# c0stya/trre

Measured on AMD Instinct MI355X. Metric: input GB/s (scan mode), higher is better.
Workload: dtype u8; 1 GPU; '[a:A-z:Z]' DFT scan over 8.000 GiB of synthetic printable lines per GPU (BASELINE.json configs[1] at north_star's size: >= 8 GiB); pattern=[a:A-z:Z], engine=dft, corpus=printable, bytes_per_gpu=8589934592, output_bytes_per_gpu=8589934592, kernel=bytemap, parallelism=line-sharded x1, one rank per GPU, no data-path collective

## Files before the change

### trre_amd/csrc/front.hpp

```cpp
#pragma once
#include <array>
#include <cstdint>
#include <memory>
#include <stdexcept>
#include <string>
#include <vector>

namespace trre {

enum : int {
    kOk = 0,
    kErrSyntax = -1,
    kErrUndefined = -2,
    kErrEpsCycle = -3,
    kErrTooBig = -4,
    kErrUnsupported = -5,
    kErrDevice = -6,
    kErrArg = -7,
    kErrDiverges = -8,
    kErrCapacity = -9
};

struct Error : std::runtime_error {
    int code;
// ... 118 lines not shown
private:
    struct Impl;
    std::unique_ptr<Impl> impl_;
};

struct StreamLimits {
    size_t max_states = 16384;
    size_t max_pending = 64;
    size_t max_out = 4096;
};
struct StreamTables {
    bool ok = false;
    bool bounded = false;
    uint32_t n_states = 0, n_cls = 0, flags = 0, max_out = 0;
    std::array<uint8_t, 256> cls{};
    std::vector<uint64_t> ent;
    std::vector<uint8_t> pool;
    std::vector<uint32_t> pending_len;
    bool lpw_ok = false;
    uint32_t lpw_delay = 0;
    std::vector<uint32_t> lpw;
    bool lpw2_ok = false;
    std::vector<uint32_t> lpw2;
    bool g16_ok = false;
    std::vector<uint32_t> g16;
    std::vector<uint32_t> mg;
    uint32_t mg_max = 0;
    bool p32_ok = false, p32_slow = false;
    std::vector<uint32_t> p32;
    bool fb_ok = false;
    uint32_t fb_states = 0, fb_dense = 0;
    uint32_t fb_start[3][2] = {};
    std::vector<uint64_t> fb_comb;
    std::vector<uint64_t> fb_lit;
    std::vector<uint32_t> fb_esc_slot;
    std::vector<uint32_t> fb_esc;
    std::vector<uint8_t> fb_pool;
    bool fb_copy_ok = false;
    std::vector<uint16_t> fb_lit_meta;
    bool fb_mark4_ok = false;
    uint32_t fb_pad = 0;
    uint32_t fb_start4[3] = {};
    std::vector<uint32_t> fb_comb4;
    std::vector<uint32_t> fb_dense4;
    std::vector<uint16_t> fb_dense_base;
};
// ... 96 lines not shown
```

### trre_amd/csrc/launch.hpp

```cpp
#pragma once
#include <cstdint>

namespace trre {

struct ScanArgs;
struct FbCopyArgs;
struct GenArgs;
struct GuardArgs;
struct LazyArgs;
struct OneArgs;
struct MapGenArgs;
struct RecArgs;
struct StrArgs;
struct MatchArgs;

constexpr int kEngineNft = 0, kEngineDft = 1;

int chunk_bytes(int engine, int mask_bytes);
int block_threads(int engine, int mask_bytes);

void launch_tile_kernel(int which, int engine, int mask_bytes, const ScanArgs& a, int64_t n_chunks, void* stream);
int direct_ent_lds_bytes();
int direct_block_threads();
void launch_direct_kernel(int which, bool ent_in_lds, const ScanArgs& a, int64_t lane_bytes, int64_t n_blocks, void* stream, int g16_bytes = 0,
                          int sym = 0, bool g16_slow = true);
int launch_one(const ScanArgs& a, const OneArgs& oa, void* stream, int g16_bytes, int sym, bool g16_slow);
int launch_mapgen(const ScanArgs& a, const MapGenArgs& oa, void* stream);
void launch_rev_sweep(const ScanArgs& a, int tab_bytes, int64_t lane_bytes, void* stream, bool packed);
void launch_rev_wide(const ScanArgs& a, int64_t lane_bytes, void* stream);
void launch_wide_fwd(int which, const ScanArgs& a, int64_t lane_bytes, int64_t n_blocks, void* stream);
void launch_lpw_kernel(int ent_bytes, bool wide, bool direct_ent_in_lds, const ScanArgs& a, int64_t lane_bytes, void* stream, int pair_bytes = 0);
void launch_fb_kernel(int which, const ScanArgs& a, const void* hdr, int64_t lane_bytes, int64_t n_chunks, void* stream);
bool fb_fits(const void* hdr);
void launch_fb_mark(const ScanArgs& a, const FbCopyArgs& ca, const void* hdr, int64_t lane_bytes, int64_t n_chunks, void* stream);
bool fb_copy_fits(const void* hdr);
void launch_fb_splice(const ScanArgs& a, const FbCopyArgs& ca, const void* hdr, int64_t lane_bytes, int64_t n_chunks, void* stream);
bool fb_splice_fits(const void* hdr);
void launch_gen(int which, const ScanArgs& a, const GenArgs& ga, int64_t lane_bytes, int64_t n_chunks, void* stream);
void launch_guard_probe(const ScanArgs& a, int64_t window, int64_t n_windows, uint64_t* flags, void* stream);
void launch_guard(bool out, const ScanArgs& a, const GuardArgs& ga, int64_t n_runs, int64_t slots, void* stream);
void launch_bt(int which, const ScanArgs& a, const GenArgs& ga, int64_t lane_bytes, int64_t n_chunks, int64_t pool_blocks, uint32_t budget, void* stream);
void launch_lazy(int which, const ScanArgs& a, const LazyArgs& la, int64_t lane_bytes, int64_t n_chunks, void* stream);
void launch_spec_verify(const ScanArgs& a, int64_t n_lanes, void* stream);
void launch_rev_verify(const ScanArgs& a, int64_t lane_bytes, void* stream, bool packed);
void launch_rev_repair(const ScanArgs& a, int64_t lane_bytes, void* stream, bool packed);
void launch_line_probe(const ScanArgs& a, int64_t window, uint32_t* out, void* stream);
void launch_chunk_scan(const uint64_t* total, uint64_t* base, int64_t n_chunks, void* stream);
void launch_bytemap(const ScanArgs& a, void* stream);
void launch_nul_eol(const uint8_t* in, int64_t n, const uint64_t* pos, uint64_t* eol, uint32_t count, void* stream);
int64_t rec_tile_bytes();
void launch_rec_check(const int64_t* off, int64_t nrec, int64_t n, uint32_t* status, void* stream);
void launch_rec_part(int side, const RecArgs& a, int64_t tiles, void* stream);
void launch_rec_stage(const RecArgs& a, int64_t tiles, void* stream);
void launch_rec_rank(const RecArgs& a, void* stream);
// ... 18 lines not shown
```

### trre_amd/csrc/runtime.cpp

```cpp
#include <hip/hip_runtime_api.h>

#include <cstdio>
#include <cstdlib>
#include <chrono>
#include <cstring>
#include <algorithm>
#include <atomic>
#include <condition_variable>
#include <functional>
#include <map>
#include <memory>
#include <mutex>
#include <string>
#include <thread>
#include <vector>

#include <sys/mman.h>

#include "../../include/trre_mi355x.h"
#include "device_blob.hpp"
#include "front.hpp"
#include "launch.hpp"
#include "switches.hpp"
#include "scan_block.hpp"
// ... 53 lines not shown
    *out = static_cast<uint8_t*>(m);
    return hipSuccess;
}
void pinned_put(uint8_t* p) {
    if (!p) return;
    size_t len = 0;
    {
        std::lock_guard<std::mutex> lk(g_pin_mu);
        auto it = g_pin_len.find(p);
        if (it == g_pin_len.end()) return;
        len = it->second;
        g_pin_len.erase(it);
    }
    (void)hipHostUnregister(p);
    ::munmap(p, len);
}

struct LaunchPlan {
    trre::ScanArgs args{};
    int64_t lane_bytes = 0, rev_lane_bytes = 0, n_chunks = 0;
    int threads = 0, sym_mode = 0;
    int g16 = 0;
    bool g16_slow = false, direct_ent_lds = false;
    bool direct = false;
    bool window = false, mapgen_on = false, use_exact = false;
};

struct Pending {
    bool active = false;
    int family = 0;
    int asked = 0;
    const uint8_t* d_in = nullptr;
    uint8_t* d_out = nullptr;
    const uint8_t* user_in = nullptr;
    bool aliased = false;
    size_t n = 0, cap = 0;
    hipStream_t stream = nullptr;
    bool launched = false;
    bool timed = false;
    int count = 0;
    const uint64_t* total_at = nullptr;
    bool patched = false;
    bool one = false;
    bool mapgen = false;
    bool exact = false;
    LaunchPlan plan;
// ... 184 lines not shown
    pred.push_back(t.to_final);
    put(b, 0, &h, 1);
    put(b, h.off_cons_mask, t.cons_mask.data(), 256);
    put(b, h.off_pred, pred.data(), pred.size());
    put(b, h.off_follow_off, t.follow_off.data(), t.follow_off.size());
    put(b, h.off_follow, t.follow.data(), t.follow.size());
    put(b, h.off_pool, t.pool.data(), t.pool.size());
}

void serialize_stream(const trre::StreamTables& t, std::vector<uint8_t>& b) {
    using namespace trre;
    StreamBlobHeader h{};
    h.magic = kMagicStream;
    h.n_states = t.n_states;
    h.n_cls = t.n_cls;
    h.flags = t.flags;
    h.max_out = t.max_out;
    size_t off = sizeof h;
    h.off_cls = (uint32_t)off; off += 256;
    h.off_ent = (uint32_t)off; h.ent_bytes = (uint32_t)(t.ent.size() * 8); off += t.ent.size() * 8;
    h.off_pool = (uint32_t)off; h.pool_bytes = (uint32_t)t.pool.size(); off += t.pool.size();
    off = align_up(off, 16);
    h.off_lpw = (uint32_t)off; h.lpw_bytes = (uint32_t)(t.lpw.size() * 4); h.lpw_delay = t.lpw_delay; off += t.lpw.size() * 4;
    off = align_up(off, 16);
    h.off_g16 = (uint32_t)off; h.g16_bytes = (uint32_t)(t.g16.size() * 4); off += t.g16.size() * 4;
    off = align_up(off, 16);
    h.off_p32 = (uint32_t)off; h.p32_bytes = (uint32_t)(t.p32.size() * 4); h.p32_slow = t.p32_slow ? 1u : 0u; off += t.p32.size() * 4;
    off = align_up(off, 16);
    h.off_lpw2 = (uint32_t)off; h.lpw2_bytes = (uint32_t)(t.lpw2.size() * 4); off += t.lpw2.size() * 4;
    off = align_up(off, 16);
    if (t.fb_ok) {
        h.fb_slots = (uint32_t)t.fb_comb.size(); h.off_fb_comb = (uint32_t)off; off = align_up(off + t.fb_comb.size() * 8, 16);
        h.fb_lits = (uint32_t)t.fb_lit.size(); h.off_fb_lit = (uint32_t)off; off = align_up(off + t.fb_lit.size() * 8, 16);
        h.fb_escs = (uint32_t)t.fb_esc_slot.size(); h.off_fb_esc_slot = (uint32_t)off; off = align_up(off + t.fb_esc_slot.size() * 4, 16);
        h.off_fb_esc = (uint32_t)off; off = align_up(off + t.fb_esc.size() * 4, 16);
        h.off_fb_pool = (uint32_t)off; off = align_up(off + t.fb_pool.size(), 16);
        if (t.fb_copy_ok) { h.off_fb_lit_meta = (uint32_t)off; off = align_up(off + t.fb_lit_meta.size() * 2, 16); }
        if (t.fb_mark4_ok) {
            h.fb4_slots = (uint32_t)t.fb_comb4.size(); h.off_fb_comb4 = (uint32_t)off; off = align_up(off + t.fb_comb4.size() * 4, 16);
            h.fb4_dense = (uint32_t)t.fb_dense_base.size(); h.off_fb_dense4 = (uint32_t)off; off = align_up(off + t.fb_dense4.size() * 4, 16);
            h.off_fb_dense_base = (uint32_t)off; off = align_up(off + t.fb_dense_base.size() * 2, 16);
            h.fb_pad = t.fb_pad;
            std::memcpy(h.fb_start4, t.fb_start4, sizeof h.fb_start4);
        }
        std::memcpy(h.fb_start, t.fb_start, sizeof h.fb_start);
    }
// ... 500 lines not shown
    pd.mapgen = true;
    return TRRE_OK;
}

int long_line_switch(trre_prog* p, ScanCtx* cx, int* family, const uint8_t* d_in, size_t n, size_t cap, hipStream_t stream) {
    const int exact_env = trre::switches().exact;
    const bool small_tables = (*family == TRRE_KERNEL_STREAM_LP && p->stt.g16_ok) || (*family == TRRE_KERNEL_GUIDED_LP && p->gt.fwd.g16_ok && !p->gt.wide);
    if (!small_tables || cx->exact_off || exact_env == 0 || cap < n) return TRRE_OK;
    if (cx->probe_in != d_in || cx->probe_n != n) {
        HIP_TRY(cx->d_probe.reserve(1, 16));
        uint32_t misses = 0;
        HIP_TRY(hipMemsetAsync(cx->d_probe, 0, 4, stream));
        trre::launch_line_probe(base_args(d_in, n), 32768, cx->d_probe, stream);
        HIP_TRY(hipMemcpyAsync(&misses, cx->d_probe, 4, hipMemcpyDeviceToHost, stream));
        HIP_TRY(hipStreamSynchronize(stream));
        cx->probe_in = d_in; cx->probe_n = n;
        cx->long_lines = misses != 0;
    }
    if (exact_env == 2 || cx->long_lines)
        *family = *family == TRRE_KERNEL_STREAM_LP ? TRRE_KERNEL_STREAM_GEN : TRRE_KERNEL_GUIDED_GEN;
    return TRRE_OK;
}

const trre::StreamTables& walked_tables(const trre_prog* p, int family) { return is_guided(family) ? p->gt.fwd : p->stt; }

LaunchPlan make_plan(const trre_prog* p, const DeviceState* st, const ScanCtx* cx, int family, const uint8_t* d_in, size_t n, uint8_t* d_out, size_t cap) {
    using namespace trre;
    const Switches& sw = switches();
    LaunchPlan pl;
    ScanArgs& args = pl.args;
    args = base_args(d_in, n, d_out);
    args.blob = is_stream(family) ? st->d_sblob : (is_guided(family) ? st->d_gblob : st->d_blob);
    const StreamTables& stt = walked_tables(p, family);
    args.status = cx->d_status;
    args.cap = cap;
    args.gscratch = cx->d_scratch.cap >= (n + 32) * (size_t)p->mask_bytes ? cx->d_scratch.p : nullptr;
    const bool backtrack = family == TRRE_KERNEL_BACKTRACK;
    const bool lazy = family == TRRE_KERNEL_DFT_LAZY;
    const int chunk = backtrack ? (int)kBtLaneBytes * 256 : lazy ? (int)kLazyLaneBytes * 256
                      : is_stream(family) ? 2048 * direct_block_threads() : chunk_bytes(p->engine, p->mask_bytes);
    pl.threads = backtrack || lazy ? 256 : is_stream(family) ? direct_block_threads() : block_threads(p->engine, p->mask_bytes);
    pl.n_chunks = (args.vend + chunk - 1) / chunk;
    pl.window = is_stream(family) && family == TRRE_KERNEL_STREAM_LP && p->stt.lpw_ok &&
                (reinterpret_cast<uintptr_t>(args.out_v0) & 15u) == 0;
    int64_t lane_auto = 2048;
    if (pl.window)
        while (lane_auto < 16384 && (int64_t)n / (lane_auto * 2) >= 524288) lane_auto *= 2;
    if ((family == TRRE_KERNEL_STREAM_GEN && (p->stt.g16_ok || p->stt.fb_ok)) || (is_guided(family) && !p->gt.wide))
        while (lane_auto < 8192 && (int64_t)n / (lane_auto * 2) >= 262144) lane_auto *= 2;
    pl.lane_bytes = sw.lane_bytes > 0 ? (sw.lane_bytes + 127) / 128 * 128 : lane_auto;
    pl.direct = is_stream(family) || is_guided(family);
    pl.rev_lane_bytes = sw.lane_bytes > 0 ? pl.lane_bytes : 2048;
    pl.direct_ent_lds = stt.ok && stt.ent.size() * 8 <= (size_t)direct_ent_lds_bytes();
    pl.g16_slow = (stt.flags & kFlagG16Slow) != 0;
    pl.g16 = stt.g16_ok && !sw.no_g16 ? (int)(align_up(stt.g16.size() * 4, 16) + stt.p32.size() * 4) : 0;
    pl.mapgen_on = stt.mg_max != 0 && (sw.mapgen < 0 ? !(stt.mg_max > 1u && cx->mapgen_dense) : sw.mapgen != 0) && !cx->mapgen_off && cx->mapgen_voids < 2;
    pl.sym_mode = !is_guided(family) ? 0 : (guided_sym_bits(*p) == 4 ? 2 : 1);
    if (pl.direct) pl.n_chunks = (args.vend + pl.lane_bytes * direct_block_threads() - 1) / (pl.lane_bytes * direct_block_threads());
    pl.use_exact = pl.g16 > 0 && !cx->exact_off && sw.exact != 0 && pl.lane_bytes % 128 == 0 && pl.rev_lane_bytes % 128 == 0 && !is_guided_wide(*p, family);
    return pl;
}


int route_lazy(trre_prog* p, DeviceState* st, ScanCtx* cx, LaunchPlan& pl, hipStream_t stream) {
    return lazy_round(p, st, cx, pl.args, pl.n_chunks, true, stream);
}
int route_backtrack(DeviceState* st, ScanCtx* cx, LaunchPlan& pl, hipStream_t stream) {
    using namespace trre;
    const BtTier& tier = kBtTiers[cx->bt_tier];
    const int64_t pool_blocks = pl.n_chunks < tier.pool_blocks ? pl.n_chunks : tier.pool_blocks;
    const uint32_t kBtFrames = tier.frames, kBtPathCap = tier.path_cap;
    const size_t need = (size_t)pool_blocks * 256 * ((size_t)kBtFrames * 16 + kBtPathCap);
    HIP_TRY(cx->d_scratch.reserve(need, need));
    GenArgs ga{};
    ga.stack = reinterpret_cast<uint32_t*>(cx->d_scratch.p);
    ga.path = cx->d_scratch + (size_t)pool_blocks * 256 * kBtFrames * 16;
    ga.frames = kBtFrames;
    ga.path_cap = kBtPathCap;
    pl.args.blob = st->d_nblob;
    const uint32_t budget = (uint32_t)switches().bt_budget.or_else(kBtBudget);
    launch_bt(1, pl.args, ga, kBtLaneBytes, pl.n_chunks, pool_blocks, budget, stream);
    launch_chunk_scan(cx->d_chunk_total, cx->d_chunk_base, pl.n_chunks, stream);
    launch_bt(2, pl.args, ga, kBtLaneBytes, pl.n_chunks, pool_blocks, budget, stream);
    return TRRE_OK;
}
int route_window(trre_prog* p, ScanCtx* cx, LaunchPlan& pl, hipStream_t stream) {
    using namespace trre;
    const int64_t n_lanes = (pl.args.vend + pl.lane_bytes - 1) / pl.lane_bytes;
    HIP_TRY(cx->d_redo.reserve((size_t)n_lanes, (size_t)(n_lanes + 1) * 4));
    HIP_TRY(hipMemsetAsync(cx->d_redo, 0, 4, stream));
    pl.args.redo = cx->d_redo;
    launch_lpw_kernel((int)(p->stt.lpw.size() * 4), p->stt.lpw_delay > 3, pl.direct_ent_lds, pl.args, pl.lane_bytes, stream,
                      p->stt.lpw2_ok && !switches().no_lpw_pair ? (int)(p->stt.lpw2.size() * 4) : 0);
    return TRRE_OK;
}
int route_wide_guided(ScanCtx* cx, LaunchPlan& pl, hipStream_t stream) {
    using namespace trre;
    launch_rev_wide(pl.args, pl.lane_bytes, stream);
    launch_wide_fwd(1, pl.args, pl.lane_bytes, pl.n_chunks, stream);
    launch_chunk_scan(cx->d_chunk_total, cx->d_chunk_base, pl.n_chunks, stream);
    launch_wide_fwd(2, pl.args, pl.lane_bytes, pl.n_chunks, stream);
    return TRRE_OK;
}
int route_lp_direct(trre_prog* p, int family, LaunchPlan& pl, hipStream_t stream) {
    using namespace trre;
    if (is_guided(family)) launch_rev_sweep(pl.args, (int)p->gt.n_rev * 256, pl.rev_lane_bytes, stream, pl.sym_mode == 2);
    pl.args.lp_emit = 1;
    launch_direct_kernel(2, pl.direct_ent_lds, pl.args, pl.lane_bytes, pl.n_chunks, stream, pl.g16, pl.sym_mode, pl.g16_slow);
    return TRRE_OK;
}
int route_large_table_copy(trre_prog* p, ScanCtx* cx, LaunchPlan& pl, hipStream_t stream) {
    using namespace trre;
    const Switches& sw = switches();
    uint32_t esc_max = 0;
    for (size_t k = 0; k + 3 < p->stt.fb_esc.size(); k += 4) esc_max = std::max(esc_max, p->stt.fb_esc[k + 1]);
    if (sw.no_fb_copy || sw.fb_emit || cx->patch_off || p->copy_form_off.load() || pl.lane_bytes % 64 != 0 || !fb_copy_fits(p->sblob.data()) ||
// ... 113 lines not shown
            hipStream_t stream) {
    Pending& pd = cx->pend;
    const bool batch = pd.active && pd.launched;
    if (pd.active && (pd.asked != family || pd.user_in != d_in || pd.d_out != d_out || pd.n != n || pd.cap != cap || pd.stream != stream))
        return fail(TRRE_E_ARG, "error: a different scan is still in flight on this device: call trre_scan_finish first");
    const int batch_count = batch ? pd.count : 0;
    const uint8_t* const user_in = d_in;
    const bool aliased = n && d_in == d_out;
    if (aliased) {
        const size_t a0 = reinterpret_cast<uintptr_t>(d_in) & 15u;
        if (!batch) {
            HIP_TRY(cx->d_snap.reserve(n + 16, n + 16));
            HIP_TRY(hipMemcpyAsync(cx->d_snap + a0, d_in, n, hipMemcpyDeviceToDevice, stream));
        }
        d_in = cx->d_snap + a0;
    }
    pd = Pending();
    pd.active = true;
    pd.count = batch_count;
    pd.family = family; pd.asked = family;
    pd.d_in = d_in; pd.d_out = d_out; pd.n = n; pd.cap = cap; pd.stream = stream;
    pd.user_in = user_in; pd.aliased = aliased;
    if (n == 0) return TRRE_OK;
    int rc = long_line_switch(p, cx, &family, d_in, n, cap, stream);
    if (rc) return rc;
    pd.family = family;
    if (family == TRRE_KERNEL_DFT_LAZY) { rc = lazy_ensure(p); if (rc) return rc; }
    LaunchPlan pl = make_plan(p, st, cx, family, d_in, n, d_out, cap);
    if (!is_gen(family) && cap < n) return TRRE_OK;
    if (is_gen(family)) {
        rc = ensure_workspace(cx, pl.n_chunks, pl.direct ? trre::direct_block_threads() : pl.threads);
        if (rc) return rc;
        pl.args.lane_counts = cx->d_lane_counts;
        pl.args.chunk_total = cx->d_chunk_total;
        pl.args.chunk_base = cx->d_chunk_base;
    }
    if (is_guided(family)) {
        const size_t need = ((size_t)((pl.args.vend + 63) & ~(int64_t)63) + 256) * (p->gt.wide ? 2 : 1);
        HIP_TRY(cx->d_sym.reserve(need, need));
        pl.args.rblob = st->d_rblob;
        pl.args.sym_v0 = cx->d_sym;
    }
    if (!batch) {
        HIP_TRY(hipMemsetAsync(cx->d_status, 0, 24, stream));
        if (p->profiling) HIP_TRY(hipEventRecord(cx->ev0, stream));
    }
    pd.timed = p->profiling;
// ... 1749 lines not shown
```

### trre_amd/csrc/scan_block.hpp

```cpp
#pragma once
#include <cstddef>
#include <cstdint>
#include <type_traits>

#include "device_blob.hpp"
#include "scan_core.hpp"

namespace trre {

struct alignas(16) U128 { uint32_t x, y, z, w; };


template <int THREADS_, int CHUNK_, int HALO_>
struct Geometry {
    static constexpr int THREADS = THREADS_;
    static constexpr int CHUNK = CHUNK_;
    static constexpr int HALO = HALO_;
    static constexpr int PRE = 16;
    static constexpr int TILE = PRE + CHUNK + HALO;
    static constexpr int TILE_ALLOC = TILE + 16;
    static constexpr int SUB = CHUNK / THREADS;
    static_assert(CHUNK % THREADS == 0 && TILE % 16 == 0, "geometry");
};

// ... 1710 lines not shown
    const uint32_t k = atomicAdd(a.redo, 1u);
#else
    const uint32_t k = a.redo[0]++;
#endif
    a.redo[1 + k] = (uint32_t)lane;
}

constexpr int kWtBlocks = 4;
constexpr int kWtPiece = 16 * kWtBlocks;
constexpr int kWtTile = 64 * kWtPiece;
constexpr int kWtOutRow = 128;
constexpr int kWtOutTile = 64 * kWtOutRow;

struct WtOutRow {
    uint8_t* row;
    uint32_t swz16;
    TRRE_HD uint8_t* slot(int b) const { return row + ((uint32_t)(b << 4) ^ swz16); }
};

TRRE_HD void lpw_classes(const LpwView& T, uint32_t w, uint32_t (&kk)[4]) {
    kk[0] = T.cls[w & 0xffu]; kk[1] = T.cls[(w >> 8) & 0xffu]; kk[2] = T.cls[(w >> 16) & 0xffu]; kk[3] = T.cls[w >> 24];
}

template <bool kCheckEnd, bool kWide>
TRRE_HD void wt_block(const LpwView& T, const U128& cur, uint32_t next_w, uint32_t (&kk)[4], int32_t rv, int32_t rhi, uint32_t& row,
                      uint32_t& win, uint32_t& win_hi, uint32_t& seen, uint32_t (&Rm)[4], uint32_t& done, int32_t& rend) {
    const uint32_t wd[5] = {cur.x, cur.y, cur.z, cur.w, next_w};
    uint32_t R = 0;
#pragma unroll
    for (int d = 0; d < 4; ++d) {
        uint32_t w = wd[d];
        const uint32_t kc[4] = {kk[0], kk[1], kk[2], kk[3]};
        lpw_classes(T, wd[d + 1], kk);
#pragma unroll
        for (int j = 0; j < 4; ++j) {
            const uint8_t* ep = reinterpret_cast<const uint8_t*>(T.ent) + row + (kc[j] << (kWide ? 5 : 4));
            const U128 e = *reinterpret_cast<const U128*>(ep);
            const uint32_t seq = perm_b32(w, e.z, e.w);
            if (!kWide) {
                win |= seq << (e.y & 63u);
                R = alignbit_b32(win, R, 8);
                win >>= 8;
            } else {
                const uint64_t e2 = *reinterpret_cast<const uint64_t*>(ep + 16);
                const uint32_t seq2 = perm_b32(w, (uint32_t)e2, (uint32_t)(e2 >> 32));
                uint64_t w64 = (uint64_t)win_hi << 32 | win;
                w64 |= ((uint64_t)seq2 << 32 | seq) << (e.y & 63u);
                R = alignbit_b32((uint32_t)w64, R, 8);
                w64 >>= 8;
                win = (uint32_t)w64;
                win_hi = (uint32_t)(w64 >> 32);
            }
            row = e.x;
            seen |= e.y;
            if (kCheckEnd) {
                const int32_t p1 = rv + 4 * d + j + 1;
                const uint32_t hit = ((e.y >> 6) & 1u) & (uint32_t)(p1 >= rhi) & (done ^ 1u);
                rend = hit ? p1 : rend;
                done |= hit;
            }
            w >>= 8;
        }
        Rm[d] = R;
        TRRE_PIN(seen);
        if (kCheckEnd) { TRRE_PIN(done); TRRE_PIN(rend); }
        TRRE_SCHED_FENCE();
    }
}

template <bool kCheckEnd>
TRRE_HD void wt_block_pair(const LpwView& T, const U128& cur, uint32_t next_w, uint32_t (&kk)[4], int32_t rv, int32_t rhi, uint32_t& row,
                           uint32_t& win, uint32_t& win_hi, uint32_t& seen, uint32_t (&Rm)[4], uint32_t& done, int32_t& rend) {
    const uint32_t wd[5] = {cur.x, cur.y, cur.z, cur.w, next_w};
    uint32_t R = 0;
#pragma unroll
    for (int d = 0; d < 4; ++d) {
        const uint32_t w = wd[d];
        const uint32_t kc[4] = {kk[0], kk[1], kk[2], kk[3]};
        lpw_classes(T, wd[d + 1], kk);
#pragma unroll
        for (int j = 0; j < 2; ++j) {
#if defined(__HIP_DEVICE_COMPILE__)
            const uint32_t col = __umul24(kc[2 * j], T.n_cls) + kc[2 * j + 1];
#else
            const uint32_t col = kc[2 * j] * T.n_cls + kc[2 * j + 1];
#endif
            const uint8_t* ep = reinterpret_cast<const uint8_t*>(T.ent) + row + (col << 5);
            const U128 e = *reinterpret_cast<const U128*>(ep);
            const uint64_t e2 = *reinterpret_cast<const uint64_t*>(ep + 16);
            const uint32_t w2 = w >> (16 * j);
            win |= perm_b32(w2, e.z, e.w);
            win_hi |= perm_b32(w2, (uint32_t)e2, (uint32_t)(e2 >> 32));
            R = alignbit_b32(win, R, 16);
            win = alignbit_b32(win_hi, win, 16);
            win_hi >>= 16;
            row = e.x;
            seen |= e.y;
            if (kCheckEnd) {
                const int32_t p1 = rv + 4 * d + 2 * j + 1;
// ... 542 lines not shown
```

### trre_amd/csrc/scan_kernels.hip

```cpp
#include <hip/hip_runtime.h>

#include <atomic>
#include <cstdlib>

#include "launch.hpp"
#include "switches.hpp"
#include "scan_block.hpp"
#include "splice_block.hpp"
#include "one_block.hpp"
#include "gen_block.hpp"
#include "lazy_block.hpp"
#include "guard_block.hpp"
#include "records_block.hpp"
#include "pass_block.hpp"

namespace trre {
namespace {

template <class G, class Engine>
struct Carve {
    static constexpr int kTab = (Engine::kLdsBytes + 15) & ~15;
    static constexpr int kMask = G::TILE_ALLOC * Engine::kMaskBytes;
    static constexpr int off_tin = 0;
    static constexpr int off_tout = G::TILE_ALLOC;
    static constexpr int off_tab = 2 * G::TILE_ALLOC;
    static constexpr int off_mask = off_tab + kTab;
    static constexpr int off_red = off_mask + ((kMask + 15) & ~15);
    static constexpr int kBytes = off_red + 64 + 16 * 8;
};

// ... 769 lines not shown
    const int64_t n_lanes = (a.vend + lane_bytes - 1) / lane_bytes;
    const dim3 grid((unsigned)((n_lanes + kWtThreads - 1) / kWtThreads));
    const bool pair = pair_bytes > 0 && pair_bytes <= kWtEntMax && !wide;
    const bool ent_in_lds = pair || ent_bytes <= kWtEntMax;
    const int ent_room = pair ? (pair_bytes + 15) / 16 * 16 : (ent_in_lds ? (ent_bytes + 15) / 16 * 16 : 0);
    const int lds = 256 + ent_room + kWtWaves * (kWtTile + kWtOutTile);
    if (pair) {
        allow_big_lds<&k_stream_lpw<true, false, true>>();
        hipLaunchKernelGGL((k_stream_lpw<true, false, true>), grid, dim3(kWtThreads), lds, s, a, lane_bytes, ent_room);
    } else if (ent_in_lds && wide) {
        allow_big_lds<&k_stream_lpw<true, true>>();
        hipLaunchKernelGGL((k_stream_lpw<true, true>), grid, dim3(kWtThreads), lds, s, a, lane_bytes, ent_room);
    } else if (ent_in_lds) {
        allow_big_lds<&k_stream_lpw<true, false>>();
        hipLaunchKernelGGL((k_stream_lpw<true, false>), grid, dim3(kWtThreads), lds, s, a, lane_bytes, ent_room);
    } else if (wide) {
        hipLaunchKernelGGL((k_stream_lpw<false, true>), grid, dim3(kWtThreads), lds, s, a, lane_bytes, ent_room);
    } else {
        hipLaunchKernelGGL((k_stream_lpw<false, false>), grid, dim3(kWtThreads), lds, s, a, lane_bytes, ent_room);
    }
    const bool ring_lds = reinterpret_cast<const void*>(a.blob) != nullptr && direct_ent_in_lds;
    if (ring_lds) hipLaunchKernelGGL((k_stream_redo<true>), dim3(64), dim3(kDirectThreads), kDirectLds, s, a, lane_bytes);
    else hipLaunchKernelGGL((k_stream_redo<false>), dim3(64), dim3(kDirectThreads), kDirectLdsHot, s, a, lane_bytes);
}
template <int kMode, bool kSym>
void launch_direct_t(bool ent_lds, const ScanArgs& a, int64_t lane_bytes, int64_t n_blocks, hipStream_t s) {
    if (ent_lds) hipLaunchKernelGGL((k_stream_direct<kMode, true, kSym>), dim3((unsigned)n_blocks), dim3(kDirectThreads), kDirectLds, s, a, lane_bytes);
    else hipLaunchKernelGGL((k_stream_direct<kMode, false, kSym>), dim3((unsigned)n_blocks), dim3(kDirectThreads), kDirectLdsHot, s, a, lane_bytes);
}
int direct_ent_lds_bytes() { return kDirectEntBytes; }
int direct_block_threads() { return kDirectThreads; }
template <int kSym, bool kHasSlow>
void launch_g16(int which, const ScanArgs& a, int64_t lane_bytes, int64_t n_blocks, hipStream_t s, int g16_bytes) {
    const int room = (g16_bytes + 15) / 16 * 16;
    const int lds = 256 + room + kDirectPoolSmall + kDirectThreads * kRingStride + 64 + kDirectWsc;
    const int lds_count = 256 + room + 64;
    allow_big_lds<&k_stream_g16<1, kSym, kHasSlow>>();
    allow_big_lds<&k_stream_g16<2, kSym, kHasSlow>>();
    if (which == 1) hipLaunchKernelGGL((k_stream_g16<1, kSym, kHasSlow>), dim3((unsigned)n_blocks), dim3(kDirectThreads), lds_count, s, a, lane_bytes, room);
    else hipLaunchKernelGGL((k_stream_g16<2, kSym, kHasSlow>), dim3((unsigned)n_blocks), dim3(kDirectThreads), lds, s, a, lane_bytes, room);
}
struct OneTailArgs {
    uint8_t* out;
    uint64_t cap;
    uint32_t* status;
    uint64_t *desc, *gsum, *ginc, *total;
// ... 843 lines not shown
```

### trre_amd/csrc/stream_pack.cpp

```cpp
#include "stream_pack.hpp"

#include <algorithm>
#include <unordered_map>

namespace trre {
namespace {

void build_window_form(StreamTables& t, const StreamPackInput& in) {
    uint32_t delay = 0;
    for (uint32_t s = 0; s < t.n_states; ++s) delay = std::max(delay, t.pending_len[s]);
    if (delay > 7) return;
    const bool wide = delay > 3;
    const uint32_t words = wide ? 8u : 4u;
    if ((size_t)t.n_states * t.n_cls * words * 4 > 32768) return;
    std::vector<uint32_t> v((size_t)t.n_states * t.n_cls * words, 0);
    for (uint32_t s = 0; s < t.n_states; ++s) {
        for (uint32_t k = 0; k < t.n_cls; ++k) {
            const StreamCell& x = in.rows[s][k];
            const size_t n = x.out.size() + (x.copy_c ? 1 : 0);
            if (n > (wide ? 8u : 4u)) return;
            uint32_t* e = &v[((size_t)s * t.n_cls + k) * words];
            e[0] = x.next * t.n_cls * words * 4u;
            const bool silent = s == in.skip || s == in.done;
            e[1] = (silent ? 0u : 8u * (delay - t.pending_len[s])) | (x.eol ? 64u : 0u) |
// ... 45 lines not shown
                uint32_t* e = &v[((size_t)s * C * C + (size_t)k0 * C + k1) * 8];
                e[0] = (uint32_t)(b.next * C * C * 32u);
                e[1] = (a.eol ? 64u : 0u) | (b.eol ? 512u : 0u) | ((a.diverge || b.diverge) ? 256u : 0u) |
                       (((in.col_kind[k0] == kColNul && !silent_a) || (in.col_kind[k1] == kColNul && !silent_b)) ? 128u : 0u);
                for (int half = 0; half < 2; ++half) {
                    uint32_t bytes = 0, sel = 0;
                    for (int i = 0; i < 4; ++i) {
                        const int w = what[4 * half + i];
                        uint32_t pick = 0x0cu;
                        if (w >= 256) pick = 4u + (uint32_t)(w - 256);
                        else if (w >= 0) { bytes |= (uint32_t)w << (8 * i); pick = (uint32_t)i; }
                        sel |= pick << (8 * i);
                    }
                    e[2 + 2 * half] = bytes;
                    e[3 + 2 * half] = sel;
                }
            }
        }
    }
    t.lpw2 = std::move(v);
    t.lpw2_ok = true;
}

void build_gen16(StreamTables& t, const StreamPackInput& in) {
    if ((size_t)t.n_states * t.n_cls > 2048) return;
    std::vector<uint32_t> v((size_t)t.n_states * t.n_cls * 4, 0);
    for (uint32_t s = 0; s < t.n_states; ++s) {
        for (uint32_t k = 0; k < t.n_cls; ++k) {
            const StreamCell& x = in.rows[s][k];
            const size_t n = x.out.size() + (x.copy_c ? 1 : 0);
            const bool slow = n > 4;
            if (slow) t.flags |= kFlagG16Slow;
            uint32_t* e = &v[((size_t)s * t.n_cls + k) * 4];
            e[0] = x.next * t.n_cls * 16u;
            const bool silent = s == in.skip || s == in.done;
            const bool ident = (x.out.empty() && x.copy_c) || (in.col_kind[k] == kColNewline && !x.copy_c && x.out == "\n");
            e[1] = (slow ? 128u : (uint32_t)n) | (x.eol ? 32u : 0u) | (x.ovf ? 64u : 0u) | (x.diverge ? 16u : 0u) |
                   ((in.col_kind[k] == kColNul && !silent) ? 8u : 0u) | (ident && !x.ovf && !x.diverge ? 256u : 512u) |
                   (silent ? 1024u : 0u) | (!silent && !(ident && !x.ovf && !x.diverge) ? 2048u : 0u) |
                   (((uint32_t)(int32_t)((slow ? 0 : (int)n) - 1) & 0xffu) << 16) |
                   ((slow ? 0u : 8u * (uint32_t)n) << 24);
            uint32_t bytes = 0, sel = 0x0c0c0c0cu;
            if (!slow) {
                sel = 0;
                for (size_t b = 0; b < 4; ++b) {
                    uint32_t pick = 0x0cu;
// ... 98 lines not shown
            if (x.diverge) lo |= 1ull << 31;
            if (nul_col && s != in.skip && s != in.done) lo |= 1ull << 29;
            if (!nul_col) {
                const size_t nl = x.out.find('\n');
                if (nl != std::string::npos && !(x.eol && nl + 1 == x.out.size())) inplace_ok = false;
                if (x.copy_c && in.col_kind[k] == kColNewline) inplace_ok = false;
            }
            t.ent[(size_t)s * t.n_cls + k] = lo | hi << 32;
            t.max_out = std::max<uint32_t>(t.max_out, (uint32_t)x.out.size() + (x.copy_c ? 1 : 0));
            if (s != in.skip && s != in.done && !nul_col && !x.diverge) {
                const int64_t emitted = (int64_t)x.out.size() + (x.copy_c ? 1 : 0);
                const int64_t expect = (int64_t)t.pending_len[s] + 1 - (int64_t)t.pending_len[x.next];
                if (emitted != expect) lp = false;
            }
        }
    }
    while (t.pool.size() % 4) t.pool.push_back(0);
    for (int k = 0; k < 8; ++k) t.pool.push_back(0);
    t.ok = true;
    t.bounded = in.bounded;
    if (in.bounded) lp = false;
    if (lp && !in.wide_cols) build_window_form(t, in);
    if (lp && !in.wide_cols) build_window_pair_form(t, in);
    if (!in.wide_cols) build_gen16(t, in);
    if (!in.wide_cols) build_pairs(t, in);
    if (lp) t.flags |= kFlagLengthPreserving;
    if (lp && inplace_ok) t.flags |= kFlagNoOverrun;
    return t;
}

}
```

### trre_amd/csrc/switches.hpp

```cpp
#pragma once
#include <cstdlib>

namespace trre {

struct SwitchNum {
    bool set = false;
    long long v = 0;
    long long or_else(long long unset) const { return set ? v : unset; }
};

inline bool switch_on(const char* v) { return v != nullptr; }
inline int switch_int(const char* v, int unset) { return v ? atoi(v) : unset; }
inline SwitchNum switch_wide(const char* v) { return v ? SwitchNum{true, atoll(v)} : SwitchNum{}; }
inline SwitchNum switch_narrow(const char* v) { return v ? SwitchNum{true, atoi(v)} : SwitchNum{}; }

struct Switches {
    bool trace = switch_on(getenv("TRRE_TRACE"));
    bool no_stack_guard = switch_on(getenv("TRRE_NO_STACK_GUARD"));
    SwitchNum guard_budget = switch_wide(getenv("TRRE_GUARD_BUDGET"));
    SwitchNum guard_call_budget = switch_wide(getenv("TRRE_GUARD_CALL_BUDGET"));
    SwitchNum lazy_budget = switch_wide(getenv("TRRE_LAZY_BUDGET"));
    SwitchNum bt_budget = switch_wide(getenv("TRRE_BT_BUDGET"));
    int exact = switch_int(getenv("TRRE_EXACT"), -1);
    long long lane_bytes = switch_wide(getenv("TRRE_LANE_BYTES")).v;
    bool no_g16 = switch_on(getenv("TRRE_NO_G16"));
    bool no_fb = switch_on(getenv("TRRE_NO_FB"));
    bool fb_emit = switch_on(getenv("TRRE_FB_EMIT"));
    bool no_fb_copy = switch_on(getenv("TRRE_NO_FB_COPY"));
    bool no_fb_mark4 = switch_on(getenv("TRRE_NO_FB_MARK4"));
    bool no_lpw_pair = switch_on(getenv("TRRE_NO_LPW_PAIR"));
    int mapgen = switch_int(getenv("TRRE_MAPGEN"), -1);
    const char* mapgen_dbg = getenv("TRRE_MAPGEN_DBG");
    int mapgen_window = switch_int(getenv("TRRE_MAPGEN_WINDOW"), 0);
    bool mapgen_nolb = switch_on(getenv("TRRE_MAPGEN_NOLB"));
    bool mapgen_prof = switch_on(getenv("TRRE_MAPGEN_PROF"));
    int mapgen_oversub = switch_int(getenv("TRRE_MAPGEN_OVERSUB"), 0);
    int one = switch_int(getenv("TRRE_ONE"), 0);
    int one_lane = switch_int(getenv("TRRE_ONE_LANE"), 0);
    int one_region = switch_int(getenv("TRRE_ONE_REGION"), 0);
    int one_look = switch_int(getenv("TRRE_ONE_LOOK"), 0);
    bool one_prof = switch_on(getenv("TRRE_ONE_PROF"));
    bool no_nul_repair = switch_on(getenv("TRRE_NO_NUL_REPAIR"));
    bool gen_host = switch_on(getenv("TRRE_GEN_HOST"));
    bool no_pinned_direct = switch_on(getenv("TRRE_NO_PINNED_DIRECT"));
    int shards_per_device = switch_int(getenv("TRRE_SHARDS_PER_DEVICE"), 1);
};

inline const Switches& switches() {
    static const Switches s;
    return s;
}

inline SwitchNum lazy_max_bytes_now() { return switch_wide(getenv("TRRE_LAZY_MAX_BYTES")); }
// ... 6 lines not shown
```

Before: 3089 GB/s.

## Add synchronizing-window kernel that scans independent 64-byte lanes without redo pass

At pack time, computes whether the length-preserving window DFA synchronizes: whether every pair of reachable states merges within a bounded number of symbols. When it does, a new kernel gives each lane a short warm-up from the preceding bytes and processes 64-byte slices independently. Tiles are staged through LDS with swizzled rows and written back with nontemporal stores, and a small end kernel handles the head and tail bytes. This removes the lane-boundary redo/fixup pass and the long-line switch. The cost is extra table analysis at build time and some redundant warm-up work per lane.

```diff
diff --git a/trre_amd/csrc/front.hpp b/trre_amd/csrc/front.hpp
--- a/trre_amd/csrc/front.hpp
+++ b/trre_amd/csrc/front.hpp
@@ -164,6 +164,7 @@
     std::vector<uint32_t> lpw;
     bool lpw2_ok = false;
     std::vector<uint32_t> lpw2;
+    uint32_t lpw_sync = 0;
     bool g16_ok = false;
     std::vector<uint32_t> g16;
     std::vector<uint32_t> mg;
diff --git a/trre_amd/csrc/launch.hpp b/trre_amd/csrc/launch.hpp
--- a/trre_amd/csrc/launch.hpp
+++ b/trre_amd/csrc/launch.hpp
@@ -30,6 +30,7 @@
 void launch_rev_wide(const ScanArgs& a, int64_t lane_bytes, void* stream);
 void launch_wide_fwd(int which, const ScanArgs& a, int64_t lane_bytes, int64_t n_blocks, void* stream);
 void launch_lpw_kernel(int ent_bytes, bool wide, bool direct_ent_in_lds, const ScanArgs& a, int64_t lane_bytes, void* stream, int pair_bytes = 0);
+bool launch_lpd_kernel(int ent_bytes, bool wide, const ScanArgs& a, void* stream, int pair_bytes = 0);
 void launch_fb_kernel(int which, const ScanArgs& a, const void* hdr, int64_t lane_bytes, int64_t n_chunks, void* stream);
 bool fb_fits(const void* hdr);
 void launch_fb_mark(const ScanArgs& a, const FbCopyArgs& ca, const void* hdr, int64_t lane_bytes, int64_t n_chunks, void* stream);
diff --git a/trre_amd/csrc/runtime.cpp b/trre_amd/csrc/runtime.cpp
--- a/trre_amd/csrc/runtime.cpp
+++ b/trre_amd/csrc/runtime.cpp
@@ -99,6 +99,7 @@
     int threads = 0, sym_mode = 0;
     int g16 = 0;
     bool g16_slow = false, direct_ent_lds = false;
+    bool lpd = false;
     bool direct = false;
     bool window = false, mapgen_on = false, use_exact = false;
 };
@@ -329,6 +330,7 @@
     h.off_pool = (uint32_t)off; h.pool_bytes = (uint32_t)t.pool.size(); off += t.pool.size();
     off = align_up(off, 16);
     h.off_lpw = (uint32_t)off; h.lpw_bytes = (uint32_t)(t.lpw.size() * 4); h.lpw_delay = t.lpw_delay; off += t.lpw.size() * 4;
+    h.pad4[0] = t.lpw_sync;
     off = align_up(off, 16);
     h.off_g16 = (uint32_t)off; h.g16_bytes = (uint32_t)(t.g16.size() * 4); off += t.g16.size() * 4;
     off = align_up(off, 16);
@@ -875,6 +877,12 @@
     return TRRE_OK;
 }
 
+bool lpd_route(const trre_prog* p, int family, const uint8_t* d_in, const uint8_t* d_out) {
+    const trre::Switches& sw = trre::switches();
+    return family == TRRE_KERNEL_STREAM_LP && p->stt.lpw_ok && p->stt.lpw_sync != 0 && sw.exact < 0 && !sw.no_lpd &&
+           ((reinterpret_cast<uintptr_t>(d_out) - reinterpret_cast<uintptr_t>(d_in)) & 15u) == 0;
+}
+
 const trre::StreamTables& walked_tables(const trre_prog* p, int family) { return is_guided(family) ? p->gt.fwd : p->stt; }
 
 LaunchPlan make_plan(const trre_prog* p, const DeviceState* st, const ScanCtx* cx, int family, const uint8_t* d_in, size_t n, uint8_t* d_out, size_t cap) {
@@ -896,6 +904,7 @@
     pl.n_chunks = (args.vend + chunk - 1) / chunk;
     pl.window = is_stream(family) && family == TRRE_KERNEL_STREAM_LP && p->stt.lpw_ok &&
                 (reinterpret_cast<uintptr_t>(args.out_v0) & 15u) == 0;
+    pl.lpd = pl.window && lpd_route(p, family, d_in, d_out);
     int64_t lane_auto = 2048;
     if (pl.window)
         while (lane_auto < 16384 && (int64_t)n / (lane_auto * 2) >= 524288) lane_auto *= 2;
@@ -939,12 +948,18 @@
 }
 int route_window(trre_prog* p, ScanCtx* cx, LaunchPlan& pl, hipStream_t stream) {
     using namespace trre;
+    const int pair_bytes = p->stt.lpw2_ok && !switches().no_lpw_pair ? (int)(p->stt.lpw2.size() * 4) : 0;
+    if (pl.lpd && launch_lpd_kernel((int)(p->stt.lpw.size() * 4), p->stt.lpw_delay > 3, pl.args, stream, pair_bytes)) {
+        if (switches().trace) fprintf(stderr, "trre: window route: k_stream_lpd (definite table, order %u)\n", p->stt.lpw_sync - 1);
+        return TRRE_OK;
+    }
+    pl.lpd = false;
+    if (switches().trace) fprintf(stderr, "trre: window route: k_stream_lpw (order %d)\n", (int)p->stt.lpw_sync - 1);
     const int64_t n_lanes = (pl.args.vend + pl.lane_bytes - 1) / pl.lane_bytes;
     HIP_TRY(cx->d_redo.reserve((size_t)n_lanes, (size_t)(n_lanes + 1) * 4));
     HIP_TRY(hipMemsetAsync(cx->d_redo, 0, 4, stream));
     pl.args.redo = cx->d_redo;
-    launch_lpw_kernel((int)(p->stt.lpw.size() * 4), p->stt.lpw_delay > 3, pl.direct_ent_lds, pl.args, pl.lane_bytes, stream,
-                      p->stt.lpw2_ok && !switches().no_lpw_pair ? (int)(p->stt.lpw2.size() * 4) : 0);
+    launch_lpw_kernel((int)(p->stt.lpw.size() * 4), p->stt.lpw_delay > 3, pl.direct_ent_lds, pl.args, pl.lane_bytes, stream, pair_bytes);
     return TRRE_OK;
 }
 int route_wide_guided(ScanCtx* cx, LaunchPlan& pl, hipStream_t stream) {
@@ -1104,7 +1119,7 @@
     pd.d_in = d_in; pd.d_out = d_out; pd.n = n; pd.cap = cap; pd.stream = stream;
     pd.user_in = user_in; pd.aliased = aliased;
     if (n == 0) return TRRE_OK;
-    int rc = long_line_switch(p, cx, &family, d_in, n, cap, stream);
+    int rc = lpd_route(p, family, d_in, d_out) ? TRRE_OK : long_line_switch(p, cx, &family, d_in, n, cap, stream);
     if (rc) return rc;
     pd.family = family;
     if (family == TRRE_KERNEL_DFT_LAZY) { rc = lazy_ensure(p); if (rc) return rc; }
diff --git a/trre_amd/csrc/scan_block.hpp b/trre_amd/csrc/scan_block.hpp
--- a/trre_amd/csrc/scan_block.hpp
+++ b/trre_amd/csrc/scan_block.hpp
@@ -1756,13 +1756,13 @@
     kk[0] = T.cls[w & 0xffu]; kk[1] = T.cls[(w >> 8) & 0xffu]; kk[2] = T.cls[(w >> 16) & 0xffu]; kk[3] = T.cls[w >> 24];
 }
 
-template <bool kCheckEnd, bool kWide>
+template <bool kCheckEnd, bool kWide, int kDwords = 4>
 TRRE_HD void wt_block(const LpwView& T, const U128& cur, uint32_t next_w, uint32_t (&kk)[4], int32_t rv, int32_t rhi, uint32_t& row,
                       uint32_t& win, uint32_t& win_hi, uint32_t& seen, uint32_t (&Rm)[4], uint32_t& done, int32_t& rend) {
     const uint32_t wd[5] = {cur.x, cur.y, cur.z, cur.w, next_w};
     uint32_t R = 0;
 #pragma unroll
-    for (int d = 0; d < 4; ++d) {
+    for (int d = 0; d < kDwords; ++d) {
         uint32_t w = wd[d];
         const uint32_t kc[4] = {kk[0], kk[1], kk[2], kk[3]};
         lpw_classes(T, wd[d + 1], kk);
@@ -1802,13 +1802,13 @@
     }
 }
 
-template <bool kCheckEnd>
+template <bool kCheckEnd, int kDwords = 4>
 TRRE_HD void wt_block_pair(const LpwView& T, const U128& cur, uint32_t next_w, uint32_t (&kk)[4], int32_t rv, int32_t rhi, uint32_t& row,
                            uint32_t& win, uint32_t& win_hi, uint32_t& seen, uint32_t (&Rm)[4], uint32_t& done, int32_t& rend) {
     const uint32_t wd[5] = {cur.x, cur.y, cur.z, cur.w, next_w};
     uint32_t R = 0;
 #pragma unroll
-    for (int d = 0; d < 4; ++d) {
+    for (int d = 0; d < kDwords; ++d) {
         const uint32_t w = wd[d];
         const uint32_t kc[4] = {kk[0], kk[1], kk[2], kk[3]};
         lpw_classes(T, wd[d + 1], kk);
diff --git a/trre_amd/csrc/scan_kernels.hip b/trre_amd/csrc/scan_kernels.hip
--- a/trre_amd/csrc/scan_kernels.hip
+++ b/trre_amd/csrc/scan_kernels.hip
@@ -6,6 +6,7 @@
 #include "launch.hpp"
 #include "switches.hpp"
 #include "scan_block.hpp"
+#include "window_block.hpp"
 #include "splice_block.hpp"
 #include "one_block.hpp"
 #include "gen_block.hpp"
@@ -821,6 +822,115 @@
     const bool ring_lds = reinterpret_cast<const void*>(a.blob) != nullptr && direct_ent_in_lds;
     if (ring_lds) hipLaunchKernelGGL((k_stream_redo<true>), dim3(64), dim3(kDirectThreads), kDirectLds, s, a, lane_bytes);
     else hipLaunchKernelGGL((k_stream_redo<false>), dim3(64), dim3(kDirectThreads), kDirectLdsHot, s, a, lane_bytes);
+}
+constexpr int kLpdThreads = 512;
+constexpr int kLpdWaves = kLpdThreads / kWave;
+constexpr int kLpdS = 64;
+constexpr int kLpdTile = kWave * kLpdS;
+constexpr int kLpdBlocksPerCu = 3;
+
+template <bool kWide, bool kPair>
+__global__ __launch_bounds__(kLpdThreads) void k_stream_lpd(ScanArgs a, int64_t first, int64_t n_tiles, int ent_room) {
+    extern __shared__ __attribute__((aligned(16))) uint8_t smem[];
+    constexpr int kBlocks = kLpdS / 16;
+    const StreamBlobHeader& h = *reinterpret_cast<const StreamBlobHeader*>(a.blob);
+    for (int k = threadIdx.x; k < 256; k += kLpdThreads) smem[k] = a.blob[h.off_cls + k];
+    const uint32_t off_ent = kPair ? h.off_lpw2 : h.off_lpw, ent_bytes = kPair ? h.lpw2_bytes : h.lpw_bytes;
+    {
+        const U128* e = reinterpret_cast<const U128*>(a.blob + off_ent);
+        U128* d = reinterpret_cast<U128*>(smem + 256);
+        for (int k = threadIdx.x; k < (int)(ent_bytes / 16); k += kLpdThreads) d[k] = e[k];
+    }
+    __syncthreads();
+    LpwView T;
+    T.cls = smem;
+    T.ent = reinterpret_cast<const U128*>(smem + 256);
+    T.delay = h.lpw_delay;
+    T.n_cls = h.n_cls;
+    const int lid = threadIdx.x & (kWave - 1), wid = threadIdx.x / kWave;
+    uint8_t* tile = smem + 256 + ent_room + wid * kLpdTile;
+    const uint32_t t0 = __builtin_amdgcn_readfirstlane(wt_lds_addr(tile));
+    const int moff = lpd_move_off<kLpdS>(lid);
+    const LpdRow<kLpdS> mine(tile, lid), below(tile, lid > 0 ? lid - 1 : 0), above(tile, lid < kWave - 1 ? lid + 1 : kWave - 1);
+    typedef uint32_t u32x4 __attribute__((ext_vector_type(4)));
+    uint32_t seen = 0;
+    const uint32_t sync = h.pad4[0];
+    const int64_t n_waves = (int64_t)gridDim.x * kLpdWaves;
+    for (int64_t t = (int64_t)blockIdx.x * kLpdWaves + wid; t < n_tiles; t += n_waves) {
+        const uint8_t* gin = a.in_v0 + first + t * kLpdTile;
+        uint8_t* gout = a.out_v0 + first + t * kLpdTile;
+        TRRE_WAIT_LGKM0();
+#pragma unroll
+        for (int i = 0; i < kBlocks; ++i) wt_glds16(gin + moff + i * 1024, t0 + i * 1024);
+        U128 warm{};
+        uint32_t f0 = 0, f1 = 0;
+        if (lid == 0) warm = *reinterpret_cast<const U128*>(gin - 16);
+        if (lid == kWave - 1) { f0 = *reinterpret_cast<const uint32_t*>(gin + kLpdTile); f1 = *reinterpret_cast<const uint32_t*>(gin + kLpdTile + 4); }
+        TRRE_WAIT_VM(0);
+        U128 b[kBlocks], o[kBlocks];
+#pragma unroll
+        for (int q = 0; q < kBlocks; ++q) b[q] = mine.load(q);
+        const U128 wb = below.load(kBlocks - 1), fa = above.load(0);
+        if (lid != 0) warm = wb;
+        if (lid != kWave - 1) { f0 = fa.x; f1 = fa.y; }
+        lpd_lane<kWide, kPair, kBlocks>(T, sync, warm, b, f0, f1, o, seen);
+#pragma unroll
+        for (int q = 0; q < kBlocks; ++q) mine.store(q, o[q]);
+#pragma unroll
+        for (int i = 0; i < kBlocks; ++i) {
+            const u32x4 ov = *reinterpret_cast<const u32x4*>(tile + i * 1024 + lid * 16);
+            u32x4* dst = reinterpret_cast<u32x4*>(gout + moff + i * 1024);
+            __builtin_nontemporal_store(ov, dst);
+        }
+    }
+    if (seen & kLpwNul) atomicOr(a.status, kStNul);
+    if (seen & kLpwDiv) atomicOr(a.status, kStDiverge);
+}
+template <bool kWide>
+__global__ __launch_bounds__(256) void k_stream_lpd_ends(ScanArgs a, LpdSpan sp) {
+    const StreamBlobHeader& h = *reinterpret_cast<const StreamBlobHeader*>(a.blob);
+    LpwView T;
+    T.cls = a.blob + h.off_cls;
+    T.ent = reinterpret_cast<const U128*>(a.blob + h.off_lpw);
+    T.delay = h.lpw_delay;
+    T.n_cls = h.n_cls;
+    const int64_t n = lpd_end_segments(a, sp);
+    uint32_t st = 0;
+    for (int64_t k = (int64_t)blockIdx.x * 256 + threadIdx.x; k < n; k += (int64_t)gridDim.x * 256) lpd_end_segment<kWide>(a, T, sp, k, st);
+    if (st) atomicOr(a.status, st);
+}
+bool launch_lpd_kernel(int ent_bytes, bool wide, const ScanArgs& a, void* stream, int pair_bytes) {
+    hipStream_t s = static_cast<hipStream_t>(stream);
+    const bool pair = pair_bytes > 0 && pair_bytes <= kWtEntMax && !wide;
+    if (!pair && ent_bytes > kWtEntMax) return false;
+    const int ent_room = ((pair ? pair_bytes : ent_bytes) + 15) / 16 * 16;
+    const int lds = 256 + ent_room + kLpdWaves * kLpdTile;
+    const LpdSpan sp = lpd_span(a.vbeg, a.vend, kLpdTile, 128);
+    if (sp.n_tiles) {
+        static std::atomic<int> cus_cache{0};
+        if (!cus_cache.load()) {
+            int dev = 0;
+            (void)hipGetDevice(&dev);
+            hipDeviceProp_t prop;
+            cus_cache.store(hipGetDeviceProperties(&prop, dev) == hipSuccess && prop.multiProcessorCount > 0 ? prop.multiProcessorCount : 256);
+        }
+        const int64_t want = (sp.n_tiles + kLpdWaves - 1) / kLpdWaves, most = (int64_t)cus_cache.load() * kLpdBlocksPerCu;
+        const dim3 grid((unsigned)(want < most ? want : most));
+        if (pair) {
+            allow_big_lds<&k_stream_lpd<false, true>>();
+            hipLaunchKernelGGL((k_stream_lpd<false, true>), grid, dim3(kLpdThreads), lds, s, a, sp.first, sp.n_tiles, ent_room);
+        } else if (wide) {
+            allow_big_lds<&k_stream_lpd<true, false>>();
+            hipLaunchKernelGGL((k_stream_lpd<true, false>), grid, dim3(kLpdThreads), lds, s, a, sp.first, sp.n_tiles, ent_room);
+        } else {
+            allow_big_lds<&k_stream_lpd<false, false>>();
+            hipLaunchKernelGGL((k_stream_lpd<false, false>), grid, dim3(kLpdThreads), lds, s, a, sp.first, sp.n_tiles, ent_room);
+        }
+    }
+    const dim3 egrid((unsigned)((lpd_end_segments(a, sp) + 255) / 256));
+    if (wide) hipLaunchKernelGGL((k_stream_lpd_ends<true>), egrid, dim3(256), 0, s, a, sp);
+    else hipLaunchKernelGGL((k_stream_lpd_ends<false>), egrid, dim3(256), 0, s, a, sp);
+    return true;
 }
 template <int kMode, bool kSym>
 void launch_direct_t(bool ent_lds, const ScanArgs& a, int64_t lane_bytes, int64_t n_blocks, hipStream_t s) {
diff --git a/trre_amd/csrc/stream_pack.cpp b/trre_amd/csrc/stream_pack.cpp
--- a/trre_amd/csrc/stream_pack.cpp
+++ b/trre_amd/csrc/stream_pack.cpp
@@ -91,6 +91,50 @@
     t.lpw2_ok = true;
 }
 
+void build_window_sync(StreamTables& t, const StreamPackInput& in) {
+    if (!t.lpw_ok) return;
+    const uint32_t n = t.n_states, C = t.n_cls;
+    std::vector<uint32_t> cols;
+    for (uint32_t k = 0; k < C; ++k)
+        if (in.col_kind[k] != kColNul) cols.push_back(k);
+    std::vector<char> reach(n, 0);
+    std::vector<uint32_t> live{0};
+    reach[0] = 1;
+    for (size_t i = 0; i < live.size(); ++i)
+        for (uint32_t k : cols) {
+            const uint32_t x = in.rows[live[i]][k].next;
+            if (!reach[x]) { reach[x] = 1; live.push_back(x); }
+        }
+    if ((in.skip < n && reach[in.skip]) || (in.done < n && reach[in.done])) return;
+    const size_t m = live.size();
+    std::vector<uint32_t> idx(n, 0);
+    for (size_t i = 0; i < m; ++i) idx[live[i]] = (uint32_t)i;
+    std::vector<uint8_t> ord(m * m, 0xff);
+    size_t open = m * (m - 1) / 2;
+    uint32_t order = 0;
+    for (uint32_t r = 1; r <= 16 && open; ++r) {
+        std::vector<size_t> now;
+        for (size_t i = 0; i < m; ++i)
+            for (size_t j = i + 1; j < m; ++j) {
+                if (ord[i * m + j] != 0xff) continue;
+                bool all = true;
+                for (uint32_t k : cols) {
+                    uint32_t a = idx[in.rows[live[i]][k].next], b = idx[in.rows[live[j]][k].next];
+                    if (a == b) continue;
+                    if (a > b) std::swap(a, b);
+                    if (ord[(size_t)a * m + b] == 0xff) { all = false; break; }
+                }
+                if (all) now.push_back(i * m + j);
+            }
+        if (now.empty()) return;
+        for (size_t q : now) ord[q] = (uint8_t)r;
+        open -= now.size();
+        order = r;
+    }
+    if (open) return;
+    t.lpw_sync = order + 1;
+}
+
 void build_gen16(StreamTables& t, const StreamPackInput& in) {
     if ((size_t)t.n_states * t.n_cls > 2048) return;
     std::vector<uint32_t> v((size_t)t.n_states * t.n_cls * 4, 0);
@@ -235,6 +279,7 @@
     if (in.bounded) lp = false;
     if (lp && !in.wide_cols) build_window_form(t, in);
     if (lp && !in.wide_cols) build_window_pair_form(t, in);
+    if (lp && !in.wide_cols) build_window_sync(t, in);
     if (!in.wide_cols) build_gen16(t, in);
     if (!in.wide_cols) build_pairs(t, in);
     if (lp) t.flags |= kFlagLengthPreserving;
diff --git a/trre_amd/csrc/switches.hpp b/trre_amd/csrc/switches.hpp
--- a/trre_amd/csrc/switches.hpp
+++ b/trre_amd/csrc/switches.hpp
@@ -29,6 +29,7 @@
     bool no_fb_copy = switch_on(getenv("TRRE_NO_FB_COPY"));
     bool no_fb_mark4 = switch_on(getenv("TRRE_NO_FB_MARK4"));
     bool no_lpw_pair = switch_on(getenv("TRRE_NO_LPW_PAIR"));
+    bool no_lpd = switch_on(getenv("TRRE_NO_LPD"));
     int mapgen = switch_int(getenv("TRRE_MAPGEN"), -1);
     const char* mapgen_dbg = getenv("TRRE_MAPGEN_DBG");
     int mapgen_window = switch_int(getenv("TRRE_MAPGEN_WINDOW"), 0);
diff --git a/trre_amd/csrc/window_block.hpp b/trre_amd/csrc/window_block.hpp
--- /dev/null
+++ b/trre_amd/csrc/window_block.hpp
@@ -0,0 +1,131 @@
+#pragma once
+#include "scan_block.hpp"
+
+namespace trre {
+
+constexpr int kLpdWarm = 16;
+constexpr int kLpdEndSeg = 16;
+
+struct LpdSpan {
+    int64_t first, n_tiles, head_end, tail_beg;
+};
+TRRE_HD LpdSpan lpd_span(int64_t vbeg, int64_t vend, int64_t tile, int64_t align) {
+    LpdSpan s;
+    s.first = (vbeg + kLpdWarm + align - 1) / align * align;
+    const int64_t room = vend - 1 - 16 - s.first;
+    s.n_tiles = room >= tile ? room / tile : 0;
+    s.head_end = s.n_tiles ? s.first : vend;
+    s.tail_beg = s.n_tiles ? s.first + s.n_tiles * tile : vend;
+    return s;
+}
+
+template <bool kWide, bool kPair, int kBlocks>
+TRRE_HD void lpd_lane(const LpwView& T, uint32_t sync, const U128& warm, const U128 (&b)[kBlocks], uint32_t flush0, uint32_t flush1,
+                      U128 (&out)[kBlocks], uint32_t& seen) {
+    const uint32_t D = T.delay & 3u;
+    uint32_t kk[4], Rm[4], row = 0, win = 0, win_hi = 0, done = 0, junk = 0, Rprev = 0;
+    int32_t rend = 0;
+    if (sync <= 5u) {
+        const U128 wu{warm.w, b[0].x, 0u, 0u};
+        lpw_classes(T, wu.x, kk);
+        if (kPair) wt_block_pair<false, 1>(T, wu, b[0].x, kk, 0, 0, row, win, win_hi, junk, Rm, done, rend);
+        else wt_block<false, kWide, 1>(T, wu, b[0].x, kk, 0, 0, row, win, win_hi, junk, Rm, done, rend);
+    } else if (sync <= 9u) {
+        const U128 wu{warm.z, warm.w, b[0].x, 0u};
+        lpw_classes(T, wu.x, kk);
+        if (kPair) wt_block_pair<false, 2>(T, wu, b[0].x, kk, 0, 0, row, win, win_hi, junk, Rm, done, rend);
+        else wt_block<false, kWide, 2>(T, wu, b[0].x, kk, 0, 0, row, win, win_hi, junk, Rm, done, rend);
+    } else {
+        lpw_classes(T, warm.x, kk);
+        if (kPair) wt_block_pair<false>(T, warm, b[0].x, kk, 0, 0, row, win, win_hi, junk, Rm, done, rend);
+        else wt_block<false, kWide>(T, warm, b[0].x, kk, 0, 0, row, win, win_hi, junk, Rm, done, rend);
+    }
+#pragma unroll
+    for (int q = 0; q < kBlocks; ++q) {
+        const uint32_t next_w = q + 1 < kBlocks ? b[(q + 1) % kBlocks].x : flush0;
+        if (kPair) wt_block_pair<false>(T, b[q], next_w, kk, 0, 0, row, win, win_hi, seen, Rm, done, rend);
+        else wt_block<false, kWide>(T, b[q], next_w, kk, 0, 0, row, win, win_hi, seen, Rm, done, rend);
+        if (q > 0) {
+            if (!kWide) {
+                out[q - 1].w = alignbyte_b32(Rm[0], Rprev, D);
+            } else {
+                out[q - 1].z = alignbyte_b32(Rm[0], Rprev, D);
+                out[q - 1].w = alignbyte_b32(Rm[1], Rm[0], D);
+            }
+        }
+        if (!kWide) {
+            out[q].x = alignbyte_b32(Rm[1], Rm[0], D);
+            out[q].y = alignbyte_b32(Rm[2], Rm[1], D);
+            out[q].z = alignbyte_b32(Rm[3], Rm[2], D);
+        } else {
+            out[q].x = alignbyte_b32(Rm[2], Rm[1], D);
+            out[q].y = alignbyte_b32(Rm[3], Rm[2], D);
+        }
+        Rprev = Rm[3];
+    }
+    const U128 fl{flush0, flush1, 0u, 0u};
+    if (kPair) wt_block_pair<false, 1>(T, fl, flush1, kk, 0, 0, row, win, win_hi, junk, Rm, done, rend);
+    else wt_block<false, kWide, kWide ? 2 : 1>(T, fl, flush1, kk, 0, 0, row, win, win_hi, junk, Rm, done, rend);
+    if (!kWide) {
+        out[kBlocks - 1].w = alignbyte_b32(Rm[0], Rprev, D);
+    } else {
+        out[kBlocks - 1].z = alignbyte_b32(Rm[0], Rprev, D);
+        out[kBlocks - 1].w = alignbyte_b32(Rm[1], Rm[0], D);
+    }
+}
+
+template <int kS>
+struct LpdRow {
+    uint8_t* row;
+    uint32_t swz16;
+    TRRE_HD static uint32_t swz_of(int r) { return kS == 64 ? (uint32_t)((r >> 1) & 3) << 4 : (uint32_t)(r & (kS / 16 - 1)) << 4; }
+    TRRE_HD LpdRow(uint8_t* tile, int r) : row(tile + r * kS), swz16(swz_of(r)) {}
+    TRRE_HD U128 load(int b) const { return *reinterpret_cast<const U128*>(row + ((uint32_t)(b << 4) ^ swz16)); }
+    TRRE_HD void store(int b, const U128& v) const { *reinterpret_cast<U128*>(row + ((uint32_t)(b << 4) ^ swz16)) = v; }
+};
+template <int kS>
+TRRE_HD int lpd_move_off(int lid) {
+    constexpr int per_row = kS / 16;
+    const int r = lid / per_row, slot = lid % per_row;
+    return r * kS + (int)(((uint32_t)(slot << 4)) ^ LpdRow<kS>::swz_of(r));
+}
+
+template <bool kWide>
+TRRE_HD void lpd_ends_walk(const ScanArgs& a, const LpwView& T, int64_t lo, int64_t hi, uint32_t& status) {
+    const int64_t delay = (int64_t)T.delay;
+    int64_t p = lo - kLpdWarm;
+    if (p < a.vbeg) p = a.vbeg;
+    uint32_t row = 0, seen = 0;
+    uint64_t win = 0;
+    for (; p < hi + delay; ++p) {
+        const uint32_t c = p >= a.vend - 1 ? (uint32_t)'\n' : (uint32_t)a.in_v0[p];
+        const uint8_t* ep = reinterpret_cast<const uint8_t*>(T.ent) + row + ((uint32_t)T.cls[c] << (kWide ? 5 : 4));
+        const U128 e = *reinterpret_cast<const U128*>(ep);
+        uint64_t seq = perm_b32(c, e.z, e.w);
+        if (kWide) {
+            const uint64_t e2 = *reinterpret_cast<const uint64_t*>(ep + 16);
+            seq |= (uint64_t)perm_b32(c, (uint32_t)e2, (uint32_t)(e2 >> 32)) << 32;
+        }
+        win |= seq << (e.y & 63u);
+        const int64_t q = p - delay;
+        if (q >= lo) a.out_v0[q] = (uint8_t)win;
+        win >>= 8;
+        row = e.x;
+        if (p >= lo && p < hi) seen |= e.y;
+    }
+    if (seen & kLpwNul) status |= kStNul;
+    if (seen & kLpwDiv) status |= kStDiverge;
+}
+TRRE_HD int64_t lpd_end_segments(const ScanArgs& a, const LpdSpan& sp) {
+    return (sp.head_end - a.vbeg + kLpdEndSeg - 1) / kLpdEndSeg + (a.vend - sp.tail_beg + kLpdEndSeg - 1) / kLpdEndSeg;
+}
+template <bool kWide>
+TRRE_HD void lpd_end_segment(const ScanArgs& a, const LpwView& T, const LpdSpan& sp, int64_t k, uint32_t& status) {
+    const int64_t n_head = (sp.head_end - a.vbeg + kLpdEndSeg - 1) / kLpdEndSeg;
+    int64_t lo, hi;
+    if (k < n_head) { lo = a.vbeg + k * kLpdEndSeg; hi = lo + kLpdEndSeg < sp.head_end ? lo + kLpdEndSeg : sp.head_end; }
+    else { lo = sp.tail_beg + (k - n_head) * kLpdEndSeg; hi = lo + kLpdEndSeg < a.vend ? lo + kLpdEndSeg : a.vend; }
+    lpd_ends_walk<kWide>(a, T, lo, hi, status);
+}
+
+}
```

Measured after the change: 3076 GB/s. No clear change (-0.4%).
